# friendlymatthew/heif

Measured on AMD Instinct MI355X. Metric: Mpixels/s decoded (bit-exact) on 4032x3024 HEIC batch, higher is better.
Workload: dtype u8

## Files before the change

heif_amd/csrc/api.cpp:

```cpp
#include <hip/hip_runtime.h>

#include <algorithm>
#include <cmath>
#include <cstdlib>
#include <cstring>
#include <atomic>
#include <memory>
#include <mutex>
#include <string>
#include <thread>
#include <vector>

#include "../../include/heifgpu.h"
#include "common/desc.hpp"
#include "host/batch.hpp"
#include "host/heic_image.hpp"
#include "kernels/cabac.hpp"
#include "kernels/kernels.hpp"

using namespace hg;

struct heifgpu_image {
    ParsedImage img;
};
// ... 962 lines not shown
    b->cur = gi;
    b->loaded = true;
    BatchArgs &a = b->args;
    a = BatchArgs{};
    a.bits = b->bits.p;
    a.pics = G.pics.p;
    a.subs = b->subs.p;
    a.rbsp = nullptr;
    a.rsubs = nullptr;
    a.parse_order = b->porder.p;
    a.n_slots = int(order.size());
    a.parse_group = parse_group;
    a.seqs = G.seqs.p;
    a.sf = G.sf.p;
    a.outs = G.outs.p;
    a.recon = b->recon.p;
    a.n_pics = b->n_pics;
    a.max_width = hb.max_w;
    a.max_wctb = hb.max_wctb;
    a.max_rows = hb.max_rows;
    a.max_log2ctb = hb.max_log2ctb;
    a.lane_rows = hb.lane_rows;
    a.parse_mode = mode;
    a.solo_waves = solo_waves;
    a.xprog = nullptr;
    a.xctx = cross_rows ? b->xctx.p : nullptr;
    a.intra_stream = intra_stream_for(mode, int(hb.pics.size()), hb.has_assembly, ctx->stream) ? 1 : 0;
    a.xntu = nullptr;
    a.stream_patience_us = ctx->stream.patience_us;
    a.wpp_ring = mode == PARSE_SOLO ? (hb.max_wpp_rows > solo_waves ? 1 : 0) : hb.wpp_ring;
    a.lanes_lean = mode == PARSE_LANES
                       ? lanes_variant_for(hb.seqs.data(), hb.pics.data(), int(hb.pics.size()), a.wpp_ring)
                       : LANES_GENERAL;
    a.has_assembly = hb.has_assembly ? 1 : 0;
    a.total_rows = int(hb.rows);
    a.bytes_per_sample = hb.bps;
    a.chroma_format = hb.chroma;
    G.out_host.assign(n, OutImage{});
    if (fresh) *inout = fresh.release();
    return HEIFGPU_OK;
}

int heifgpu_batch_prepare(heifgpu_ctx *ctx, const heifgpu_image *const *imgs, size_t n, heifgpu_batch **out) {
    if (!out) return fail(HEIFGPU_E_INVALID, "invalid argument");
    *out = nullptr;
    const int rc = heifgpu_batch_prepare_ex(ctx, imgs, n, nullptr, out);
    if (rc) return rc;
    HIP_TRY(hipStreamSynchronize(ctx->upload));
    return HEIFGPU_OK;
}

int heifgpu_batch_decode(heifgpu_ctx *ctx, heifgpu_batch *b, const heifgpu_planes *out, void *stream) {
    if (!ctx || !b || !out) return fail(HEIFGPU_E_INVALID, "invalid argument");
    if (b->device != ctx->device) return fail(HEIFGPU_E_INVALID, "batch belongs to another device");
    if (!b->loaded) return fail(HEIFGPU_E_INVALID, "batch not loaded (its last prepare failed)");
    hipStream_t s = static_cast<hipStream_t>(stream);
    HIP_TRY(hipSetDevice(ctx->device));
    DescGen &G = b->gen[b->cur];
    bool changed = false;
    for (size_t i = 0; i < b->n_images; ++i) {
        OutImage o{};
        for (int c = 0; c < 3; ++c) {
            o.plane[c] = reinterpret_cast<uint64_t>(out[i].plane[c]);
            o.pitch[c] = out[i].pitch[c];
        }
        if (!out[i].plane[0] || (b->infos[i].chroma_format_idc && (!out[i].plane[1] || !out[i].plane[2])))
// ... 357 lines not shown
```

heif_amd/csrc/emu/emu_check.cpp:

```cpp
#include <cstdio>
#include <cstdlib>
#include <cstring>
#include <vector>

#include "../../../oracle/oracle.h"
#include "../host/batch.hpp"
#include "../kernels/cabac.hpp"
#include "../kernels/kernels.hpp"

namespace hg {
thread_local EmuCtx g_emu;
}
using namespace hg;

int main(int argc, char **argv) {
    if (argc < 2) return 2;
    setvbuf(stdout, nullptr, _IONBF, 0);
    int stages = argc > 2 ? atoi(argv[2]) : 5;
    const bool host_only = stages <= 0;
    const uint32_t tstride = !host_only && argc > 4 ? uint32_t(atoi(argv[3])) : 1u,
                   toff = !host_only && argc > 4 ? uint32_t(atoi(argv[4])) : 0u;
    auto read_file = [](const char *path, std::vector<uint8_t> &out) {
        FILE *f = fopen(path, "rb");
        if (!f) return false;
// ... 1 lines not shown
        long n = ftell(f);
        fseek(f, 0, SEEK_SET);
        out.assign(static_cast<size_t>(n), 0);
        const bool ok = fread(out.data(), 1, size_t(n), f) == size_t(n);
        fclose(f);
        return ok;
    };
    std::vector<uint8_t> data;
    if (!read_file(argv[1], data)) return 2;
    std::vector<std::vector<uint8_t>> more_data;
    for (int k = 3; host_only && k < argc; ++k) {
        more_data.emplace_back();
        if (!read_file(argv[k], more_data.back())) return 2;
    }
    ParsedImage im;
    std::vector<ParsedImage> more(more_data.size());
    HostBatch hb;
    try {
        im = parse_heic(data.data(), data.size());
        std::vector<const ParsedImage *> ims{&im};
        for (size_t k = 0; k < more.size(); ++k) {
            more[k] = parse_heic(more_data[k].data(), more_data[k].size());
            ims.push_back(&more[k]);
        }
        hb = build_batch(ims.data(), ims.size(), tstride, toff);
    } catch (const std::exception &e) {
        printf("host rejected: %s\n", e.what());
        return 3;
    }
    std::vector<TuRec> tus(hb.tu_n);
    std::vector<Coef> coefs(hb.coef_n);
    std::vector<uint32_t> rc(2 * hb.rows), status(hb.pics.size());
    std::vector<uint8_t> recon(hb.recon_bytes), maps(hb.map_bytes);
    std::vector<int16_t> resid(hb.resid_elems);
    std::vector<SaoParams> sao(hb.sao_n);
    const int W = int(im.out_width), H = int(im.out_height), bps = hb.bps;
    const int SX = chroma_sx(hb.chroma), SY = chroma_sy(hb.chroma);
    const int CW = (W + (1 << SX) - 1) >> SX, CH = (H + (1 << SY) - 1) >> SY;
    constexpr uint8_t kSentinel = 0xa5;
    std::vector<uint8_t> oy(size_t(W) * H * bps, kSentinel), ocb(size_t(CW) * CH * bps, kSentinel),
        ocr(size_t(CW) * CH * bps, kSentinel);
    OutImage out{};
    out.plane[0] = uint64_t(oy.data());
    out.plane[1] = uint64_t(ocb.data());
    out.plane[2] = uint64_t(ocr.data());
    out.pitch[0] = W * bps;
    out.pitch[1] = out.pitch[2] = CW * bps;
    out.width = W;
    out.height = H;
    BatchArgs a{};
    a.bits = hb.bits.data();
    a.pics = hb.pics.data();
    a.subs = hb.subs.data();
    std::vector<uint8_t> rbsp(hb.bits.size(), 0);
    std::vector<uint32_t> rsubs(hb.subs.size(), 0);
    a.rbsp = rbsp.data();
    a.rsubs = rsubs.data();
    std::vector<uint32_t> order;
    const int mode = parse_mode_for(PARSE_AUTO, int(hb.pics.size()), hb.pics.data());
    const int solo_waves = solo_waves_for(hb.lane_rows);
    int parse_group = 1;
    if (mode == PARSE_SPREAD) spread_parse_order(hb.pics.data(), int(hb.pics.size()), order);
    else
        parse_group = lanes_parse_order(hb.pics.data(), int(hb.pics.size()), hb.lane_rows, mode == PARSE_SOLO ? 1 : 0,
                                        order);
    std::vector<uint32_t> xprog(hb.rows + 1), xntu(hb.rows + hb.pics.size() + 1, 0);
// ... 1 lines not shown
    a.parse_order = order.data();
    a.n_slots = int(order.size());
    a.parse_group = parse_group;
    a.seqs = hb.seqs.data();
    a.sf = hb.sf.data();
    a.outs = &out;
    a.tus = tus.data();
    a.coefs = coefs.data();
    a.row_counts = rc.data();
    a.recon = recon.data();
    a.resid = resid.data();
    a.maps = maps.data();
    a.sao = sao.data();
    a.status = status.data();
    a.n_pics = int(hb.pics.size());
    a.max_width = hb.max_w;
    a.max_wctb = hb.max_wctb;
    a.max_rows = hb.max_rows;
    a.max_log2ctb = hb.max_log2ctb;
    a.lane_rows = hb.lane_rows;
    a.parse_mode = mode;
    a.solo_waves = solo_waves;
    a.xprog = xprog.data();
    a.xctx = xctx.data();
    a.xjob = xprog.data() + hb.rows;
    const StreamKnobs knobs = stream_knobs_from_env();
    a.intra_stream = intra_stream_for(mode, int(hb.pics.size()), hb.has_assembly, knobs) ? 1 : 0;
    a.xntu = a.intra_stream ? xntu.data() : nullptr;
    a.stream_patience_us = knobs.patience_us;
    a.wpp_ring = mode == PARSE_SOLO ? (hb.max_wpp_rows > solo_waves ? 1 : 0) : hb.wpp_ring;
    a.lanes_lean = mode == PARSE_LANES
                       ? lanes_variant_for(hb.seqs.data(), hb.pics.data(), int(hb.pics.size()), a.wpp_ring)
                       : LANES_GENERAL;
    a.has_assembly = hb.has_assembly ? 1 : 0;
    a.total_rows = int(hb.rows);
    a.bytes_per_sample = bps;
    a.chroma_format = hb.chroma;
    if (stages <= 0) {
        printf("host ok: %zu pictures\n", hb.pics.size());
        printf("parse mode: %s\n", mode == PARSE_SOLO ? "solo" : mode == PARSE_SPREAD ? "spread" : "lanes");
        if (mode == PARSE_LANES) printf("lanes variant: %s\n", a.lanes_lean ? "lean" : "general");
        return 0;
    }
    std::fill(rc.begin(), rc.end(), 0xa5a5a5a5u);
    std::fill(status.begin(), status.end(), 0x5au);
    std::fill(xprog.begin(), xprog.end(), 0x7777u);
    std::fill(xntu.begin(), xntu.end(), 0x3333u);
    emu_rbsp(a);
    emu_parse(a);
    uint32_t st = 0;
    for (uint32_t s : status) st |= s;
    uint64_t ntu = 0, ncoef = 0;
    for (uint32_t r = 0; r < hb.rows; ++r) {
        ntu += rc[2 * r];
        ncoef += rc[2 * r + 1];
    }
    if (getenv("HG_EMU_DEBUG_MODES")) {
        int shown = 0;
        for (const PicDesc &pd : hb.pics)
            for (uint32_t r = 0; r < (uint32_t)((hb.seqs[pd.seq].height + (1 << hb.seqs[pd.seq].log2_ctb) - 1) >> hb.seqs[pd.seq].log2_ctb); ++r) {
                const uint32_t nt = rc[2 * (pd.row_off + r)];
                for (uint32_t t = 0; t < nt && shown < 10; ++t) {
                    const TuRec &tu = tus[pd.tu_off + (uint64_t)r * pd.tu_cap_row + t];
                    if (tu.mode > 34) {
                        printf("bad mode %d pic %u row %u t %u x %d y %d log2 %d flags 0x%x ctu %d\n", tu.mode, (unsigned)(&pd - hb.pics.data()), r, t, tu.x, tu.y, tu.log2, tu.flags, tu.ctu);
                        ++shown;
                    }
                }
            }
    }
    printf("parse mode: %s\n", mode == PARSE_SOLO     ? "solo"
                               : mode == PARSE_SPREAD ? "spread"
                                                      : "lanes");
    if (mode == PARSE_LANES) printf("lanes variant: %s\n", a.lanes_lean ? "lean" : "general");
    printf("parse: status 0x%x, %llu TBs, %llu coefficients\n", st, (unsigned long long)ntu, (unsigned long long)ncoef);
    if (stages >= 2 && !a.intra_stream) emu_transform(a);
    if (stages >= 3) {
        emu_intra(a);
        if (a.intra_stream) {
            BatchArgs a2 = a;
            a2.stream_redo = 1;
            emu_intra(a2);
        }
    }
    if (stages >= 4) emu_deblock(a);
    if (stages >= 5) {
        emu_sao_out(a);
    } else {
        int dbk = stages >= 4 ? 0 : 1;
        oracle_set_debug_flags(dbk | 2);
        for (const PicDesc &pd : hb.pics) {
            const SeqParams &sp = hb.seqs[pd.seq];
            for (int c = 0; c < 3; ++c) {
                if (c && !sp.chroma_format) break;
                const int sx = c ? SX : 0, sy = c ? SY : 0, PW = sp.width >> sx, PH = sp.height >> sy;
                size_t off = c == 0 ? 0 : size_t(sp.width) * sp.height + size_t(c - 1) * PW * PH;
                int vw = std::min(sp.out_w, W - pd.out_x) >> sx, vh = std::min(sp.out_h, H - pd.out_y) >> sy;
                for (int y = 0; y < vh; ++y)
                    for (int x = 0; x < vw; ++x) {
                        size_t src = (off + size_t(y + (sp.conf_t >> sy)) * PW + x + (sp.conf_l >> sx)) * bps;
                        uint8_t *dst = reinterpret_cast<uint8_t *>(out.plane[c]) +
                                       size_t((pd.out_y >> sy) + y) * out.pitch[c] + size_t((pd.out_x >> sx) + x) * bps;
                        memcpy(dst, recon.data() + pd.recon_off + src, size_t(bps));
                    }
            }
        }
    }
    if (stages < 3) return st ? 1 : 0;
    oracle_image ref;
    if (oracle_decode_heic(data.data(), data.size(), &ref, nullptr, 0, nullptr)) {
        printf("oracle failed: %s\n", oracle_last_error());
        return 1;
    }
    long bad_total = 0;
    const char *names[3] = {"Y", "Cb", "Cr"};
    for (int c = 0; c < 3; ++c) {
        const uint8_t *g = c == 0 ? oy.data() : (c == 1 ? ocb.data() : ocr.data());
        int pw = int(ref.pw[c]), ph = int(ref.ph[c]);
// ... 28 lines not shown
```

heif_amd/csrc/emu/emu_parse.cpp:

```cpp
#include "../kernels/parse_units.hpp"

#include <cstdio>
#include <string>
#include <vector>

namespace hg {

template <class EG>
void emu_parse_lanes(const BatchArgs &a) {
    const int ppw = a.parse_order && a.parse_group > 0 ? a.parse_group : lanes_pics_per_wave(a.lane_rows, a.n_pics);
    const int n_slots = a.parse_order ? a.n_slots : a.n_pics;
    const int waves = (n_slots + ppw - 1) / ppw;
    uint64_t tab[kTabRows], seq[15];
    uint8_t scan8[128];
    for (int i = 0; i < 64; ++i) scan8_tables(scan8, i);
    for (int i = 0; i < kTabRows; ++i) tab[i] = state_row_ctx(i);
    for (int i = 0; i < 15; ++i) seq[i] = sig_seq(i);
    std::vector<LaneLds> lds(64);
    std::vector<LanePic> pics(64);
    std::vector<Lane> lanes(64);
    std::vector<uint8_t> wctx(a.wpp_ring ? 64 * CTX_PAD : 0);
    uint32_t prog[64];
    static const bool stats = std::getenv("HEIFGPU_LANES_STATS") != nullptr;
    static const std::string order = [] {
// ... 49 lines not shown
                    HG_COV(any4 ? COV_SB_RUN_ANY4 : COV_SB_RUN_NO4);
                }
                for (int l = 0; l < 64; ++l) {
                    Lane &L = lanes[l];
                    E.lane = l;
                    LanePic &P = pics[l / a.lane_rows];
                    if (!mine[l]) continue;
                    progressed = true;
                    ++units;
                    const EG G{lds[l].ctx, tab, seq, a.rbsp, (P.bits_end + 64u) & ~3u, scan8, scan8 + 64};
                    run_unit(kind, L, lds[l], P, E, G);
                }
            }
            if (!progressed) {
                for (int l = 0; l < 64; ++l)
                    if (lanes[l].st != U_DONE) {
                        lanes[l].status |= ST_SUBSTREAM_END;
                        atomicOr(&a.status[pics[l / a.lane_rows].pic], lanes[l].status & ~ST_SEGSW);
                        lanes[l].st = U_DONE;
                    }
                break;
            }
        }
        if (stats) {
            printf("wave %d: %ld passes, %.1f units per pass, %ld kind runs, %.2f units per kind run\n", w, passes,
                   (double)units / passes, kruns, (double)units / kruns);
            printf("  runs");
            for (int k = U_CTU; k <= U_TBD; ++k) printf(" %ld", kr[k]);
            printf("\n  units");
            for (int k = U_CTU; k <= U_TBD; ++k) printf(" %ld", ku[k]);
            printf("\n  paths");
            for (int k = 0; k < COV_N; ++k) printf(" %ld", g_cov[k]), g_cov[k] = 0;
            printf("\n  sb_paths");
            for (int k = COV_N; k < COV_ALL; ++k) printf(" %ld", g_cov[k]), g_cov[k] = 0;
            printf("\n");
        }
    }
}

template <bool Spread>
void emu_parse_solo(const BatchArgs &a) {
    using EG = EngSoloT<Spread>;
    const int NW = Spread ? a.max_rows : a.solo_waves;
    const int n_slots = a.parse_order ? a.n_slots : a.n_pics;
    uint64_t seq[15];
    for (int i = 0; i < 15; ++i) seq[i] = sig_seq(i);
    std::vector<LaneLds> lds((size_t)NW);
    std::vector<Lane> lanes((size_t)NW);
    std::vector<uint8_t> wctx((size_t)NW * CTX_PAD);
    std::vector<uint32_t> wbuf((size_t)NW * 192);
    std::vector<SoloWin> wins((size_t)NW);
    LanePic P;
    uint32_t prog[64];
    for (int slot = 0; slot < n_slots; ++slot) {
        const bool in = !a.parse_order || a.parse_order[slot] != ~0u;
        if (!in) continue;
        const uint32_t ent = a.parse_order ? a.parse_order[slot] : (uint32_t)slot;
        if (Spread && (ent >> 20) != 0) continue;
        const int pic = a.pic0 + (int)(Spread ? (ent & 0xfffffu) : ent);
        for (int w = 0; w < NW; ++w) {
            prog[w] = 0;
            if (!lane_init<false>(lanes[(size_t)w], P, lds[(size_t)w], a, pic, w, 0, Spread ? (1 << 20) : NW))
                lanes[(size_t)w].st = U_DONE;
            wins[(size_t)w].w = &wbuf[(size_t)w * 192];
            wins[(size_t)w].f = &wbuf[(size_t)w * 192 + 128];
        }
        const uint32_t lim = (P.bits_end + 64u) & ~3u;
// ... 43 lines not shown
```

heif_amd/csrc/kernels/kernels.hpp:

```cpp
#pragma once
#include "../common/desc.hpp"
#include "wave.hpp"
#include <cstdlib>
#include <vector>

#if defined(HG_HOST_EMU)
#include <atomic>
#include <thread>
#endif

namespace hg {

struct BatchArgs {
    const uint8_t *bits;
    const PicDesc *pics;
    const uint32_t *subs;
    uint8_t *rbsp;
    uint32_t *rsubs;
    const uint32_t *parse_order;
    int n_slots;
    const SeqParams *seqs;
    const uint8_t *sf;
    const OutImage *outs;
    TuRec *tus;
    Coef *coefs;
    uint32_t *row_counts;
    uint8_t *recon;
    int16_t *resid;
    uint8_t *maps;
    SaoParams *sao;
    uint32_t *status;
    int n_pics;
    int pic0;
    int max_width;
    int max_wctb;
    int max_rows;
    int total_rows;
    int bytes_per_sample;
    int chroma_format;
    int parse_group;
    int max_log2ctb;
    int lane_rows;
    int wpp_ring;
    int parse_mode;
    int solo_waves;
    uint32_t *xprog;
    uint8_t *xctx;
    uint32_t *xntu;
    uint32_t *xjob;
    int intra_stream;
    int stream_redo;
    uint32_t stream_patience_us;
    int has_assembly;
    int intra_split;
    int lanes_lean;
};

struct ColorArgs {
    uint64_t plane[3];
    int32_t pitch[3];
    uint64_t rgb;
    int32_t rgb_pitch;
    int32_t w, h;
    int32_t out_w, out_h;
    int32_t rotation;
    int32_t chroma, shift;
    int32_t yoff, ys;
    int32_t cr_r, cb_g, cr_g, cb_b;
};
struct GatherArgs {
    uint64_t dst[3], src[3];
    int32_t dpitch[3], spitch[3];
    int32_t planes, bps;
    int32_t sx, sy;
    int32_t W, H;
    int32_t tw, th, cols, n_tiles, stride, offset;
};
inline void color_coefs(uint32_t matrix, bool full, ColorArgs &c) {
    double kr = 0.299, kb = 0.114;
    if (matrix == 1) kr = 0.2126, kb = 0.0722;
    else if (matrix == 9) kr = 0.2627, kb = 0.0593;
    const double kg = 1.0 - kr - kb;
    const double ys = full ? 1.0 : 255.0 / 219.0, cs = full ? 1.0 : 255.0 / 224.0;
    auto fx = [](double v) { return (int32_t)(v * 65536.0 + 0.5); };
    c.yoff = full ? 0 : 16;
    c.ys = fx(ys);
    c.cr_r = fx(2.0 * (1.0 - kr) * cs);
    c.cb_b = fx(2.0 * (1.0 - kb) * cs);
// ... 142 lines not shown
```

heif_amd/csrc/kernels/parse_state.hpp:

```cpp
#pragma once
#include "cabac.hpp"
#include "kernels.hpp"
#include "tables.hpp"

#include <algorithm>
#include <cstdint>
#include <vector>

#if defined(HG_HOST_EMU)
#include <cstdio>
#endif

#if !defined(HG_HOST_EMU)
extern "C" __device__ int hg_writelane(int src, int lane, int old) __asm("llvm.amdgcn.writelane.i32");
#endif
#if !defined(HG_NO_COLD_HINTS)
#define HG_UNLIKELY(x) __builtin_expect(!!(x), 0)
#define HG_LIKELY(x) __builtin_expect(!!(x), 1)
#else
#define HG_UNLIKELY(x) (x)
#define HG_LIKELY(x) (x)
#endif

namespace hg {
// ... 89 lines not shown

struct Lane {
    uint32_t range, value;
    int k;
    uint64_t cur;
    int cn;
    uint32_t a0, a1, a2, a3, b0, b1, b2, b3, f0, f1, f2, f3;
    int ai, bv, fp;
    uint32_t lb;
    int32_t budget;
    uint32_t status;
    int st;
    uint32_t fl;
    int row, c, ctbx, ctby;
    int qx, qy, ql, qd;
    int tx, ty, tl, td;
    uint32_t tcbf;
    int qp_prev_last, qp_pred, cu_qp_delta_val, qpy_cur, qg_x, qg_y;
    int cu_modes, cu_chroma;
    int tb_t, tb_n, tb_cidx, tb_x, tb_y, tb_log2, tb_mode;
    uint32_t tb_coef0;
    int rc_scan, rc_last_sub, rc_last_pos, rc_i, rc_prev_c1;
    uint64_t rc_csbf;
    uint32_t ntu, ncoef;
    uint32_t nesc;
    uint32_t tu_row, coef_row;
    uint32_t cx;
    uint32_t reinit;
#if defined(HG_PARSE_PROF_SB)
    uint64_t psb[6];
#endif
};
#if defined(HG_PARSE_PROF_SB) && !defined(HG_HOST_EMU)
#define HG_SB_T(L, i, t0)                                                            \
    do {                                                                             \
        const uint64_t t_ = __builtin_amdgcn_s_memtime();                            \
        if ((int)__lane_id() == __builtin_ctzll(__ballot(1))) (L).psb[i] += t_ - (t0); \
        (t0) = t_;                                                                   \
    } while (0)
#else
#define HG_SB_T(L, i, t0) ((void)0)
#endif

enum Cov : int {
    COV_TB_LUMA,
    COV_TB_CHROMA = COV_TB_LUMA + 4,
    COV_NXN = COV_TB_CHROMA + 4,
    COV_NXN_MPM,
    COV_NXN_REM = COV_NXN_MPM + 3,
    COV_DQP,
    COV_DQP_EG0,
    COV_LAST_SUFFIX,
    COV_CODED_AFTER_EMPTY,
    COV_CU_ENDS_IN_SB,
    COV_TSKIP,
    COV_LAST_CTX5,
    COV_N,
    COV_SB_SIG4 = COV_N,
    COV_SB_SIG,
    COV_SB_BEYOND8,
    COV_SB_RICE4,
    COV_SB_ESCAPE,
    COV_SB_EGK,
    COV_SB_HIDE,
    COV_SB_NO_HIDE,
    COV_SB_CTXSET_INC,
    COV_SB_INFER_DC,
    COV_SB_LAST_POS0,
    COV_SB_GT2,
    COV_SB_RUN_ANY4,
    COV_SB_RUN_NO4,
    COV_ALL
};
#if defined(HG_HOST_EMU)
long g_cov[COV_ALL];
#define HG_COV(i) (++g_cov[i])
#else
#define HG_COV(i) ((void)0)
#endif

HG_HD inline size_t lane_blocks_bytes(int n) { return (sizeof(LaneLds) * (size_t)n + 15) & ~(size_t)15; }

#if !defined(HG_HOST_EMU) && defined(HG_PARSE_PROF)
int prof_read(uint64_t *out, int n) {
    uint64_t tmp[16] = {};
    if (hipMemcpyFromSymbol(tmp, HIP_SYMBOL(hg::g_prof_lanes), sizeof(tmp)) != hipSuccess) return -1;
    const uint64_t zero[16] = {};
    if (hipMemcpyToSymbol(HIP_SYMBOL(hg::g_prof_lanes), zero, sizeof(zero)) != hipSuccess) return -1;
#if defined(HG_PARSE_PROF_SB)
    const int head = 16;
#else
    const int head = 8;
#endif
    for (int k = 0; k < n && k < head; ++k) out[k] = tmp[k];
    if (n <= head) return n < head ? n : head;
    const size_t m = std::min((size_t)(n - head), (size_t)hg::kCtuTimeCap * 3);
    if (hipMemcpyFromSymbol(out + head, HIP_SYMBOL(hg::g_ctu_t), m * sizeof(uint64_t)) != hipSuccess) return -1;
    std::vector<uint64_t> z((size_t)hg::kCtuTimeCap * 3, 0);
    if (hipMemcpyToSymbol(HIP_SYMBOL(hg::g_ctu_t), z.data(), z.size() * sizeof(uint64_t)) != hipSuccess) return -1;
    return (int)(head + m);
}
#endif

}
// ... 2 lines not shown
```

heif_amd/csrc/kernels/parse_units.hpp:

```cpp
#pragma once
#include "parse_engine.hpp"

namespace hg {
namespace {

HG_HD inline int mode422(int m) {
    constexpr uint32_t t[9] = {0x02020100u, 0x05030202u, 0x0b0a0807u, 0x12100f0du, 0x16151413u,
                               0x18181717u, 0x1b1a1919u, 0x1d1c1c1bu, 0x001f1e1du};
    return (int)((t[m >> 2] >> (8 * (m & 3))) & 0xffu);
}

HG_HD inline int chroma_qp_map(int qpi, int chroma) {
    if (chroma != 1) return qpi < 51 ? qpi : 51;
    if (qpi < 30) return qpi;
    if (qpi > 43) return qpi - 6;
    return qpi < 34 ? qpi - 1 : 33 + ((qpi - 34) >> 1);
}

HG_HD inline void update_qpy(Lane &L, const LanePic &P) {
    L.qpy_cur = ((L.qp_pred + L.cu_qp_delta_val + 52 + 2 * P.qpbdY) % (52 + P.qpbdY)) - P.qpbdY;
}

HG_HD inline void derive_qp_pred(Lane &L, const LaneLds &ld, const LanePic &P) {
    int prev;
// ... 433 lines not shown
        if (nxn) HG_COV(p ? COV_NXN_MPM + mpm : COV_NXN_REM);
        const int xPb = L.qx + (i & 1) * pb, yPb = L.qy + (i >> 1) * pb;
        const int m = derive_luma_mode(L, ld, xPb, yPb, p, mpm, rem);
        modes |= m << (8 * i);
        const int nb = pb >> 2, by = (yPb - L.ctby) >> 2, bx = (xPb - L.ctbx) >> 2;
        for (int k = 0; k < nb; ++k) {
            ld.ipmL[by + k] = (uint8_t)m;
            ld.ipmA[bx + k] = (uint8_t)m;
        }
    }
    L.cu_modes = modes;
    if (HG_PIC_CHROMA(P)) {
        const int nc = HG_PIC_CHROMA(P) == 3 ? np : 1;
        int cms = 0;
        for (int i = 0; i < nc; ++i) {
            const int icpm = dec(L, G, CTX_CHROMA_MODE) ? (int)byp_bits(L, G, 2) : 4;
            const int lm = (modes >> (8 * i)) & 0xff;
            int cm;
            if (icpm == 4) {
                cm = lm;
            } else {
                cm = icpm == 0 ? 0 : (icpm == 1 ? 26 : (icpm == 2 ? 10 : 1));
                if (cm == lm) cm = 34;
            }
            if (HG_PIC_CHROMA(P) == 2) cm = mode422(cm);
            cms |= cm << (8 * i);
        }
        L.cu_chroma = nc == 1 ? (int)((uint32_t)cms * 0x01010101u) : cms;
    }
    L.tx = L.qx, L.ty = L.qy, L.tl = L.ql, L.td = 0, L.tcbf = 0;
    L.st = U_TT;
}

template <class EG>
HG_HD inline void unit_tt(Lane &L, LaneLds &ld, LanePic &P, const EG &G) {
    const bool nxn = (L.fl & F_NXN) != 0;
    const int max_depth = P.maxDepthIntra + (nxn ? 1 : 0);
    for (;;) {
        bool split;
        if (L.tl <= P.maxTb && L.tl > P.minTb && L.td < max_depth && !(nxn && L.td == 0))
            split = dec(L, G, CTX_SPLIT_TF + 5 - L.tl) != 0;
        else
            split = L.tl > P.maxTb || (nxn && L.td == 0);
        uint32_t cbf = 0;
        if ((L.tl > 2 && HG_PIC_CHROMA(P)) || HG_PIC_CHROMA(P) == 3) {
            const uint32_t pc = L.td == 0 ? 3u : (L.tcbf >> (4 * (L.td - 1))) & 3u;
            const bool two = HG_PIC_CHROMA(P) == 2 && (!split || L.tl == 3);
            if (pc & 1) {
                cbf |= (uint32_t)dec(L, G, CTX_CBF_CHROMA + L.td);
                if (two) cbf |= (uint32_t)dec(L, G, CTX_CBF_CHROMA + L.td) << 2;
            }
            if (pc & 2) {
                cbf |= (uint32_t)dec(L, G, CTX_CBF_CHROMA + L.td) << 1;
                if (two) cbf |= (uint32_t)dec(L, G, CTX_CBF_CHROMA + L.td) << 3;
            }
        }
        L.tcbf = (L.tcbf & ~(15u << (4 * L.td))) | (cbf << (4 * L.td));
        if (!split) break;
        --L.tl;
        ++L.td;
    }
    const uint32_t cbf = (L.tcbf >> (4 * L.td)) & 15u;
    L.fl &= ~F_CBF_L;
    if (dec(L, G, CTX_CBF_LUMA + (L.td == 0 ? 1 : 0))) L.fl |= F_CBF_L;
    const bool chroma4 = (HG_PIC_CHROMA(P) == 1 || HG_PIC_CHROMA(P) == 2) && L.tl == 2;
    const uint32_t pc = L.td > 0 ? (L.tcbf >> (4 * (L.td - 1))) & 15u : 0u;
    const bool cbf_c = HG_PIC_CHROMA(P) == 0 ? false : (chroma4 ? pc != 0 : cbf != 0);
    if (((L.fl & F_CBF_L) || cbf_c) && (pic_flags<EG>(P) & SP_CU_QP_DELTA) && !(L.fl & F_DQP_CODED)) {
// ... 2 lines not shown
            v = dec(L, G, CTX_CU_QP_DELTA);
            if (v) {
                uint32_t t = ctx_ld(L, G, CTX_CU_QP_DELTA + 1);
                while (v < 5 && dec_t(L, G, t & 0x7fu, t)) ++v;
                ctx_st(L, G, CTX_CU_QP_DELTA + 1, t & 0x7fu);
            }
        } else {
            while (v < 5 && dec(L, G, CTX_CU_QP_DELTA + (v == 0 ? 0 : 1))) ++v;
        }
        HG_COV(COV_DQP);
        if (v == 5) {
            HG_COV(COV_DQP_EG0);
            int ones = 0;
            bool bad = false;
            while (byp(L, G)) {
                if (++ones > 31) {
                    bad = true;
                    break;
                }
            }
            if (bad) L.status |= ST_SYNTAX;
            else v += (int)(((1u << ones) - 1u) + byp_bits(L, G, ones));
        }
        if (v && byp(L, G)) v = -v;
        const int vlo = -(26 + P.qpbdY / 2), vhi = 25 + P.qpbdY / 2;
        if (HG_UNLIKELY(v < vlo || v > vhi)) {
            L.status |= ST_SYNTAX;
            v = v < vlo ? vlo : vhi;
        }
        L.fl |= F_DQP_CODED;
        L.cu_qp_delta_val = v;
        update_qpy(L, P);
    }
    {
        const int nb = 1 << (L.tl - 2), gx0 = L.tx >> 2, gy0 = L.ty >> 2;
        const int wx = gx0 + nb <= P.w4 ? nb : P.w4 - gx0, hy = gy0 + nb <= P.h4 ? nb : P.h4 - gy0;
        const uint64_t nf = (lane_fl<EG>(L) & F_BYPASS) ? MF_NOFILT : 0;
        const uint64_t rep = 0x0101010101010101ull;
        for (int y = 0; y < hy; ++y) {
            uint8_t *row = P.gflags + (size_t)(gy0 + y) * P.w4 + gx0;
            const uint64_t h = (y == 0 ? (uint64_t)MF_EDGE_H : 0u) | nf;
            store_bytes(row, wx, (rep * h) | (uint64_t)MF_EDGE_V);
        }
    }
    const int blk = L.td == 0 ? 0 : (((L.tx >> L.tl) & 1) | (((L.ty >> L.tl) & 1) << 1));
    L.tb_n = (HG_PIC_CHROMA(P) != 0 && (!chroma4 || blk == 3)) ? (HG_PIC_CHROMA(P) == 2 ? 5 : 3) : 1;
    L.tb_t = 0;
    L.st = U_TB;
}

template <class EG>
HG_HD inline void tu_emit(Lane &L, const LanePic &P) {
    const uint32_t fl = lane_fl<EG>(L);
    int qp;
    if (L.tb_cidx == 0) {
        qp = L.qpy_cur + P.qpbdY;
    } else {
        const int off = L.tb_cidx == 1 ? P.cbOff : P.crOff;
        int qpi = L.qpy_cur + off;
        qpi = qpi < -P.qpbdC ? -P.qpbdC : (qpi > 57 ? 57 : qpi);
        qp = chroma_qp_map(qpi, HG_PIC_CHROMA(P)) + P.qpbdC;
    }
    uint32_t f = (uint32_t)L.tb_cidx;
    if (fl & F_TB_CBF) f |= TU_CBF;
    if (fl & F_TS) f |= TU_TSKIP;
    if (fl & F_BYPASS) f |= TU_BYPASS;
    if (fl & F_PCM) f |= TU_PCM | TU_BYPASS;
    if (L.tb_cidx == 0 && L.tb_log2 == 2) f |= TU_DST;
    if (HG_LIKELY(L.ntu < P.tu_cap)) {
        const uint32_t w0 = (uint32_t)L.tb_x | ((uint32_t)L.tb_y << 16);
        const uint32_t w1 = (uint32_t)L.tb_log2 | (f << 8) | ((uint32_t)L.tb_mode << 16) | ((uint32_t)(uint8_t)qp << 24);
        const uint32_t w3 = (L.ncoef - L.tb_coef0) | ((uint32_t)L.c << 16);
        if (pic_flags<EG>(P) & PF_COHERENT) store_tu_agent(P.tu_base + L.tu_row + L.ntu, w0, w1, L.tb_coef0, w3);
        else store_tu(P.tu_base + L.tu_row + L.ntu, w0, w1, L.tb_coef0, w3);
        ++L.ntu;
    } else {
        L.status |= ST_CAPACITY;
    }
}

HG_HD inline void cu_done(Lane &L, LaneLds &ld, LanePic &P);

template <class EG>
HG_HD inline void tb_done(Lane &L, LaneLds &ld, LanePic &P) {
    tu_emit<EG>(L, P);
    if (++L.tb_t < L.tb_n) {
        L.st = U_TB;
        return;
    }
    while (L.td > 0) {
        const int s = 1 << L.tl;
        const int b = ((L.tx >> L.tl) & 1) | (((L.ty >> L.tl) & 1) << 1);
        if (b < 3) {
            const int px = L.tx & ~(2 * s - 1), py = L.ty & ~(2 * s - 1);
            L.tx = px + ((b + 1) & 1) * s;
            L.ty = py + ((b + 1) >> 1) * s;
            L.st = U_TT;
            return;
        }
        L.tx &= ~(2 * s - 1);
        L.ty &= ~(2 * s - 1);
        ++L.tl;
        --L.td;
    }
    cu_done(L, ld, P);
}

HG_HD inline void cu_done(Lane &L, LaneLds &ld, LanePic &P) {
    {
        const int n = 1 << L.ql, nd = n >> 3;
        const int dy = (L.qy - L.ctby) >> 3, dx = (L.qx - L.ctbx) >> 3;
        for (int k = 0; k < nd; ++k) {
            ld.qL[dy + k] = (int8_t)L.qpy_cur;
            ld.qA[dx + k] = (int8_t)L.qpy_cur;
        }
        const int nb = n >> 2, gx0 = L.qx >> 2, gy0 = L.qy >> 2;
        const int wx = gx0 + nb <= P.w4 ? nb : P.w4 - gx0, hy = gy0 + nb <= P.h4 ? nb : P.h4 - gy0;
        for (int y = 0; y < hy; ++y) {
            int8_t *row = P.gqpy + (size_t)(gy0 + y) * P.w4 + gx0;
            store_bytes(reinterpret_cast<uint8_t *>(row), wx, 0x0101010101010101ull * (uint8_t)L.qpy_cur);
        }
        L.qp_prev_last = L.qpy_cur;
    }
    while (L.qd > 0) {
        const int s = 1 << L.ql;
        const int px = L.qx & ~(2 * s - 1), py = L.qy & ~(2 * s - 1);
        for (int b = (((L.qx >> L.ql) & 1) | (((L.qy >> L.ql) & 1) << 1)) + 1; b < 4; ++b) {
            const int cx = px + (b & 1) * s, cy = py + (b >> 1) * s;
            if (cx < P.W && cy < P.H) {
                L.qx = cx;
                L.qy = cy;
                L.st = U_CQT;
                return;
            }
        }
        L.qx = px;
        L.qy = py;
        ++L.ql;
        --L.qd;
    }
    L.st = U_CTU_END;
}

template <class EG>
HG_HD inline void unit_tb(Lane &L, LaneLds &ld, LanePic &P, const EG &G) {
    const int t = L.tb_t;
    const bool chroma4 = (HG_PIC_CHROMA(P) == 1 || HG_PIC_CHROMA(P) == 2) && L.tl == 2;
    const bool c422 = HG_PIC_CHROMA(P) == 2;
    const int comp = t == 0 ? 0 : (c422 ? 1 + ((t - 1) >> 1) : t), half = (c422 && t > 0) ? (t - 1) & 1 : 0;
    bool cbf;
    L.tb_cidx = comp;
    if (t == 0) {
        L.tb_x = L.tx;
        L.tb_y = L.ty;
        L.tb_log2 = L.tl;
        int k = 0;
        if (L.fl & F_NXN) {
            const int half = 1 << (L.ql - 1);
            k = ((L.ty - L.qy) >= half ? 2 : 0) + ((L.tx - L.qx) >= half ? 1 : 0);
        }
        L.tb_mode = (L.cu_modes >> (8 * k)) & 0xff;
        cbf = (L.fl & F_CBF_L) != 0;
    } else if (!chroma4) {
        L.tb_log2 = HG_PIC_CHROMA(P) == 3 ? L.tl : L.tl - 1;
        L.tb_x = L.tx >> HG_PIC_SUBX(P);
        L.tb_y = (L.ty >> HG_PIC_SUBY(P)) + (half << L.tb_log2);
        int k = 0;
        if (HG_PIC_CHROMA(P) == 3 && (L.fl & F_NXN)) {
            const int hp = 1 << (L.ql - 1);
            k = ((L.ty - L.qy) >= hp ? 2 : 0) + ((L.tx - L.qx) >= hp ? 1 : 0);
        }
        L.tb_mode = (L.cu_chroma >> (8 * k)) & 0xff;
        cbf = ((L.tcbf >> (4 * L.td + (comp - 1) + 2 * half)) & 1u) != 0;
    } else {
        const int s = 1 << (L.tl + 1);
        L.tb_x = (L.tx & ~(s - 1)) >> 1;
        L.tb_y = ((L.ty & ~(s - 1)) >> HG_PIC_SUBY(P)) + 4 * half;
        L.tb_log2 = 2;
        L.tb_mode = L.cu_chroma & 0xff;
        cbf = ((L.tcbf >> (4 * (L.td - 1) + (comp - 1) + 2 * half)) & 1u) != 0;
    }
    L.fl = (L.fl & ~(F_TS | F_TB_CBF)) | (cbf ? F_TB_CBF : 0u);
    L.tb_coef0 = L.ncoef;
    if (!cbf) {
        if constexpr (EG::kSolo) tb_done<EG>(L, ld, P);
        else L.st = U_TBD;
        return;
    }
    const int l2 = L.tb_log2, n = 1 << l2, cidx = comp;
    HG_COV((cidx ? COV_TB_CHROMA : COV_TB_LUMA) + l2 - 2);
    if (t == 1 && !(L.fl & F_CBF_L)) HG_COV(COV_CODED_AFTER_EMPTY);
    if ((pic_flags<EG>(P) & SP_TRANSFORM_SKIP) && !(L.fl & F_BYPASS) && l2 == 2 && dec(L, G, CTX_TS_FLAG + (cidx ? 1 : 0)))
        L.fl |= F_TS;
    if (L.fl & F_TS) HG_COV(COV_TSKIP);
    const int cmax = (l2 << 1) - 1;
    const int off = cidx == 0 ? 3 * (l2 - 2) + ((l2 - 1) >> 2) : 15;
    const int shift = cidx == 0 ? (l2 + 1) >> 2 : l2 - 2;
    int px = 0, py = 0;
    while (px < cmax && dec(L, G, CTX_LAST_X + off + (px >> shift))) ++px;
    while (py < cmax && dec(L, G, CTX_LAST_Y + off + (py >> shift))) ++py;
    int lx = px, ly = py;
    if (px > 3 || py > 3) HG_COV(COV_LAST_SUFFIX);
    if (px > 8 || py > 8) HG_COV(COV_LAST_CTX5);
    if (px > 3) {
        const int k = (px >> 1) - 1;
        lx = (1 << k) * (2 + (px & 1)) + (int)byp_bits(L, G, k);
    }
    if (py > 3) {
        const int k = (py >> 1) - 1;
        ly = (1 << k) * (2 + (py & 1)) + (int)byp_bits(L, G, k);
    }
    int scan = 0;
    if (l2 == 2 || (l2 == 3 && (cidx == 0 || HG_PIC_CHROMA(P) == 3))) {
        if (L.tb_mode >= 6 && L.tb_mode <= 14) scan = 2;
        else if (L.tb_mode >= 22 && L.tb_mode <= 30) scan = 1;
    }
    if (scan == 2) {
        const int tt = lx;
        lx = ly;
        ly = tt;
    }
    if (HG_UNLIKELY(lx >= n || ly >= n)) {
        L.status |= ST_SYNTAX;
        lx &= n - 1;
        ly &= n - 1;
    }
    const int sbl = l2 - 2, sbw = 1 << sbl;
    L.rc_scan = scan;
    L.rc_last_sub = scan_inv(G, sbl, scan, (ly >> 2) * sbw + (lx >> 2));
    L.rc_last_pos = scan_inv(G, 2, scan, (ly & 3) * 4 + (lx & 3));
    L.rc_csbf = 0;
    L.rc_prev_c1 = 1;
    L.fl &= ~F_ANY_SB;
    L.rc_i = L.rc_last_sub;
    L.st = U_SB;
}

template <bool Scalar = false>
HG_HD inline uint64_t spread16_nib(uint32_t m) {
#if !defined(HG_HOST_EMU) && defined(__HIP_DEVICE_COMPILE__)
    if constexpr (Scalar) {
        uint64_t x2, x4;
        asm("s_bitreplicate_b64_b32 %0, %1" : "=s"(x2) : "s"(uni32(m & 0xffffu)));
        asm("s_bitreplicate_b64_b32 %0, %1" : "=s"(x4) : "s"((uint32_t)x2));
        return x4 & 0x1111111111111111ull;
    }
#endif
    uint64_t x = m & 0xffffu;
    x = (x | (x << 24)) & 0x000000ff000000ffull;
    x = (x | (x << 12)) & 0x000f000f000f000full;
    x = (x | (x << 6)) & 0x0303030303030303ull;
    x = (x | (x << 3)) & 0x1111111111111111ull;
    return x;
}

template <class EG>
constexpr bool kSbVec = !EG::kSolo;

HG_HD inline uint64_t spread16_nib_halves(uint32_t m) {
    auto half = [](uint32_t x) {
        x = (x | (x << 12)) & 0x000f000fu;
        x = (x | (x << 6)) & 0x03030303u;
        x = (x | (x << 3)) & 0x11111111u;
        return x;
    };
    return (uint64_t)half(m & 0xffu) | ((uint64_t)half((m >> 8) & 0xffu) << 32);
}

// ... 132 lines not shown
            }
            if (nstart >= 0) {
                HG_COV(l2 == 2 ? COV_SB_SIG4 : COV_SB_SIG);
                if (infer_dc && sig == 0) {
                    HG_COV(COV_SB_INFER_DC);
                    sig |= 1u;
                } else {
                    sig |= dec_slot((int)(seq & 15u));
                }
            } else {
                HG_COV(COV_SB_LAST_POS0);
            }
        }
        auto cw = [&](int i, uint32_t v) { ctx_st(L, G, cbase + i, v & 0xffu); };
        if constexpr (kCc7) {
            if (l2 == 2) {
                for (int k = 0; k < 9; ++k) cw(k, (uint32_t)(cc >> (7 * k)) & 0x7fu);
            } else {
                cw(0, (uint32_t)cc & 0x7fu);
                cw(off, (uint32_t)(cc >> 7) & 0x7fu);
                cw(off + 1, (uint32_t)(cc >> 14) & 0x7fu);
                cw(off + 2, (uint32_t)(cc >> 21) & 0x7fu);
            }
        } else if (l2 == 2) {
            for (int k = 0; k < 4; ++k) cw(k, c0 >> (8 * k));
            for (int k = 0; k < 4; ++k) cw(4 + k, c1 >> (8 * k));
            cw(8, c2);
        } else {
            cw(0, c0);
            cw(off, c0 >> 8);
            cw(off + 1, c0 >> 16);
            cw(off + 2, c0 >> 24);
        }
#if defined(HG_PARSE_PROF_SB) && !defined(HG_HOST_EMU)
        L.psb[4] += (uint64_t)(nstart + 1);
#endif
        HG_SB_T(L, 1, tsb);
    }
    if (sig) {
        int ctx_set = (i == 0 || cidx > 0) ? 0 : 2;
        if ((L.fl & F_ANY_SB) && L.rc_prev_c1 == 0) {
            HG_COV(COV_SB_CTXSET_INC);
            ++ctx_set;
        }
        L.fl |= F_ANY_SB;
        int c1 = 1;
        uint32_t g1 = 0, g2 = 0;
        const int gbase = CTX_GT1 + ctx_set * 4 + (cidx ? 16 : 0);
        uint32_t gc = ctx_ld(L, G, gbase) | (ctx_ld(L, G, gbase + 1) << 8) | (ctx_ld(L, G, gbase + 2) << 16) |
                      (ctx_ld(L, G, gbase + 3) << 24);
        const int first_sig = 31 - __builtin_clz(sig & (0u - sig));
        const int last_sig = msb32(sig);
        int num_g1 = 0, last_g1 = -1;
        uint32_t beyond8 = sig;
        if constexpr (EG::kSolo) {
            uint32_t &m = beyond8;
            for (int j = 0; j < 8 && m; ++j) {
                const int nn = msb32(m);
                m ^= 1u << nn;
                const uint32_t gs = (uint32_t)(c1 < 3 ? c1 : 3) * 8u;
                uint32_t cs = (gc >> gs) & 0xffu;
                const uint32_t f = (uint32_t)dec_s(L, G, cs);
                gc = (gc & ~(0xffu << gs)) | (cs << gs);
                g1 |= f << nn;
                c1 = (c1 > 0 && !f) ? c1 + 1 : 0;
            }
            last_g1 = g1 ? msb32(g1) : -1;
// ... 290 lines not shown
```

heif_amd/csrc/kernels/transform.hip:

```cpp
#include "xform.hpp"

namespace hg {

namespace {

#ifndef HG_XF_WAVES
#define HG_XF_WAVES 4
#endif
constexpr int kWaves = HG_XF_WAVES;

#define wave_sync() HG_WAVE_SYNC()

}

#if !defined(HG_XF_WPE)
#define HG_XF_WPE 7
#endif
__global__ void __launch_bounds__(kWaves * 64) __attribute__((amdgpu_waves_per_eu(HG_XF_WPE))) k_transform(BatchArgs a) {
    HG_BLOCK_SHARED __attribute__((aligned(16))) int16_t dtile[kWaves][32 * kXfDStride32];
    HG_BLOCK_SHARED __attribute__((aligned(16))) int16_t gtile[kWaves][32 * 32];
    HG_BLOCK_SHARED int32_t extent[kWaves][2];
    HG_BLOCK_SHARED XfTab s_tab;
#if defined(HG_HOST_EMU)
    xf_tables(&s_tab, 0, 1);
// ... 140 lines not shown
                     res_plane[cidx] + (size_t)tu.y * pitch[cidx] + tu.x, pitch[cidx], lane);
    };
    auto wanted = [&](const TuRec &tu) {
        const int cidx = tu.flags & TU_CIDX_MASK, n = 1 << tu.log2;
        return (tu.flags & TU_CBF) && tu.log2 != 2 && tu.log2 <= 5 && cidx <= 2 && tu.x + n <= pitch[cidx] &&
               tu.y + n <= (cidx ? ch : H);
    };
#if defined(HG_HOST_EMU)
    for (uint32_t t = wave; t < ntu; t += kWaves)
        if (wanted(tus[t])) pass_b(tus[t]);
#else
    for (uint32_t t0 = wave; t0 < ntu; t0 += 64u * kWaves) {
        const uint32_t t = t0 + (uint32_t)lane * kWaves;
        uint4 rec = make_uint4(0, 0, 0, 0);
        if (t < ntu) rec = *reinterpret_cast<const uint4 *>(tus + t);
        TuRec mine;
        __builtin_memcpy(&mine, &rec, sizeof(mine));
        uint64_t todo = __ballot(t < ntu && wanted(mine));
        while (todo) {
            const int j = __builtin_ctzll(todo);
            todo &= todo - 1;
            const uint4 r = make_uint4((uint32_t)__builtin_amdgcn_readlane((int)rec.x, j),
                                       (uint32_t)__builtin_amdgcn_readlane((int)rec.y, j),
                                       (uint32_t)__builtin_amdgcn_readlane((int)rec.z, j),
                                       (uint32_t)__builtin_amdgcn_readlane((int)rec.w, j));
            TuRec tu;
            __builtin_memcpy(&tu, &r, sizeof(tu));
            pass_b(tu);
        }
    }
#endif
}

#if defined(HG_HOST_EMU)
void emu_transform(const BatchArgs &a) { emu_launch(k_transform, a.max_rows, a.n_pics, kWaves, a); }
#else
hipError_t launch_transform(const BatchArgs &a, hipStream_t s) {
    hipLaunchKernelGGL(k_transform, dim3(a.max_rows, a.n_pics), dim3(kWaves * 64), 0, s, a);
    return hipGetLastError();
}
#endif

}
```

Before: 26810.

## Move deblock edge-flag painting out of lanes parser into separate kernel

In the lanes parse mode the per-TU deblocking edge/bypass flag map is no longer written inside the serial CABAC parse loop. A new kernel launched after the transform pass rebuilds those flags from the stored TU records instead. The aim is to shorten the latency-bound parse critical path by moving byte-map stores into a parallel pass. The cost is an extra kernel launch and a re-read of the TU records, and the change also adds per-TB profiling macros and coverage counters for the emulator.

```diff
diff --git a/heif_amd/csrc/api.cpp b/heif_amd/csrc/api.cpp
--- a/heif_amd/csrc/api.cpp
+++ b/heif_amd/csrc/api.cpp
@@ -1018,6 +1018,7 @@
     a.lanes_lean = mode == PARSE_LANES
                        ? lanes_variant_for(hb.seqs.data(), hb.pics.data(), int(hb.pics.size()), a.wpp_ring)
                        : LANES_GENERAL;
+    a.flags_from_recs = mode == PARSE_LANES ? 1 : 0;
     a.has_assembly = hb.has_assembly ? 1 : 0;
     a.total_rows = int(hb.rows);
     a.bytes_per_sample = hb.bps;
diff --git a/heif_amd/csrc/emu/emu_check.cpp b/heif_amd/csrc/emu/emu_check.cpp
--- a/heif_amd/csrc/emu/emu_check.cpp
+++ b/heif_amd/csrc/emu/emu_check.cpp
@@ -57,6 +57,7 @@
     std::vector<Coef> coefs(hb.coef_n);
     std::vector<uint32_t> rc(2 * hb.rows), status(hb.pics.size());
     std::vector<uint8_t> recon(hb.recon_bytes), maps(hb.map_bytes);
+    if (getenv("HEIFGPU_EMU_DUMP_MAPS")) std::fill(maps.begin(), maps.end(), uint8_t(0xa5));
     std::vector<int16_t> resid(hb.resid_elems);
     std::vector<SaoParams> sao(hb.sao_n);
     const int W = int(im.out_width), H = int(im.out_height), bps = hb.bps;
@@ -124,6 +125,7 @@
     a.lanes_lean = mode == PARSE_LANES
                        ? lanes_variant_for(hb.seqs.data(), hb.pics.data(), int(hb.pics.size()), a.wpp_ring)
                        : LANES_GENERAL;
+    a.flags_from_recs = mode == PARSE_LANES ? 1 : 0;
     a.has_assembly = hb.has_assembly ? 1 : 0;
     a.total_rows = int(hb.rows);
     a.bytes_per_sample = bps;
@@ -176,6 +178,16 @@
         }
     }
     if (stages >= 4) emu_deblock(a);
+    if (const char *path = getenv("HEIFGPU_EMU_DUMP_MAPS")) {
+        FILE *f = fopen(path, "wb");
+        if (!f) return 2;
+        for (const PicDesc &pd : hb.pics) {
+            const SeqParams &sp = hb.seqs[pd.seq];
+            const size_t n = size_t((sp.width + 3) >> 2) * size_t((sp.height + 3) >> 2);
+            fwrite(maps.data() + pd.map_off, 1, 2 * n, f);
+        }
+        fclose(f);
+    }
     if (stages >= 5) {
         emu_sao_out(a);
     } else {
diff --git a/heif_amd/csrc/emu/emu_parse.cpp b/heif_amd/csrc/emu/emu_parse.cpp
--- a/heif_amd/csrc/emu/emu_parse.cpp
+++ b/heif_amd/csrc/emu/emu_parse.cpp
@@ -105,7 +105,9 @@
             printf("\n  paths");
             for (int k = 0; k < COV_N; ++k) printf(" %ld", g_cov[k]), g_cov[k] = 0;
             printf("\n  sb_paths");
-            for (int k = COV_N; k < COV_ALL; ++k) printf(" %ld", g_cov[k]), g_cov[k] = 0;
+            for (int k = COV_N; k < COV_SB_END; ++k) printf(" %ld", g_cov[k]), g_cov[k] = 0;
+            printf("\n  tb_paths");
+            for (int k = COV_SB_END; k < COV_ALL; ++k) printf(" %ld", g_cov[k]), g_cov[k] = 0;
             printf("\n");
         }
     }
diff --git a/heif_amd/csrc/kernels/kernels.hpp b/heif_amd/csrc/kernels/kernels.hpp
--- a/heif_amd/csrc/kernels/kernels.hpp
+++ b/heif_amd/csrc/kernels/kernels.hpp
@@ -54,6 +54,7 @@
     int has_assembly;
     int intra_split;
     int lanes_lean;
+    int flags_from_recs;
 };
 
 struct ColorArgs {
diff --git a/heif_amd/csrc/kernels/parse_state.hpp b/heif_amd/csrc/kernels/parse_state.hpp
--- a/heif_amd/csrc/kernels/parse_state.hpp
+++ b/heif_amd/csrc/kernels/parse_state.hpp
@@ -145,14 +145,26 @@
 #endif
 };
 #if defined(HG_PARSE_PROF_SB) && !defined(HG_HOST_EMU)
-#define HG_SB_T(L, i, t0)                                                            \
+#define HG_PHASE_T(L, i, t0)                                                         \
     do {                                                                             \
         const uint64_t t_ = __builtin_amdgcn_s_memtime();                            \
         if ((int)__lane_id() == __builtin_ctzll(__ballot(1))) (L).psb[i] += t_ - (t0); \
         (t0) = t_;                                                                   \
     } while (0)
+#endif
+#if defined(HG_PARSE_PROF_SB) && !defined(HG_HOST_EMU) && !defined(HG_PARSE_PROF_TB)
+#define HG_SB_T(L, i, t0) HG_PHASE_T(L, i, t0)
+#elif defined(HG_PARSE_PROF_TB) && !defined(HG_HOST_EMU)
+#define HG_SB_T(L, i, t0) ((void)(t0))
 #else
 #define HG_SB_T(L, i, t0) ((void)0)
+#endif
+#if defined(HG_PARSE_PROF_TB) && !defined(HG_HOST_EMU)
+#define HG_TB_T0(t0) uint64_t t0 = __builtin_amdgcn_s_memtime()
+#define HG_TB_T(L, i, t0) HG_PHASE_T(L, i, t0)
+#else
+#define HG_TB_T0(t0) ((void)0)
+#define HG_TB_T(L, i, t0) ((void)0)
 #endif
 
 enum Cov : int {
@@ -183,6 +195,14 @@
     COV_SB_GT2,
     COV_SB_RUN_ANY4,
     COV_SB_RUN_NO4,
+    COV_SB_END,
+    COV_LAST_00 = COV_SB_END,
+    COV_LAST_0M,
+    COV_LAST_M0,
+    COV_LAST_MM,
+    COV_LAST_SUFFIX_X_ONLY,
+    COV_LAST_SUFFIX_Y_ONLY,
+    COV_LAST_SWAP,
     COV_ALL
 };
 #if defined(HG_HOST_EMU)
diff --git a/heif_amd/csrc/kernels/parse_units.hpp b/heif_amd/csrc/kernels/parse_units.hpp
--- a/heif_amd/csrc/kernels/parse_units.hpp
+++ b/heif_amd/csrc/kernels/parse_units.hpp
@@ -489,8 +489,17 @@
     L.st = U_TT;
 }
 
+#if defined(HG_FLAGS_IN_PARSE)
+template <class EG>
+constexpr bool kFlagsInParse = true;
+#else
+template <class EG>
+constexpr bool kFlagsInParse = EG::kSolo;
+#endif
+
 template <class EG>
 HG_HD inline void unit_tt(Lane &L, LaneLds &ld, LanePic &P, const EG &G) {
+    HG_TB_T0(ttt);
     const bool nxn = (L.fl & F_NXN) != 0;
     const int max_depth = P.maxDepthIntra + (nxn ? 1 : 0);
     for (;;) {
@@ -559,7 +568,8 @@
         L.cu_qp_delta_val = v;
         update_qpy(L, P);
     }
-    {
+    HG_TB_T(L, 3, ttt);
+    if constexpr (kFlagsInParse<EG>) {
         const int nb = 1 << (L.tl - 2), gx0 = L.tx >> 2, gy0 = L.ty >> 2;
         const int wx = gx0 + nb <= P.w4 ? nb : P.w4 - gx0, hy = gy0 + nb <= P.h4 ? nb : P.h4 - gy0;
         const uint64_t nf = (lane_fl<EG>(L) & F_BYPASS) ? MF_NOFILT : 0;
@@ -570,6 +580,7 @@
             store_bytes(row, wx, (rep * h) | (uint64_t)MF_EDGE_V);
         }
     }
+    HG_TB_T(L, 4, ttt);
     const int blk = L.td == 0 ? 0 : (((L.tx >> L.tl) & 1) | (((L.ty >> L.tl) & 1) << 1));
     L.tb_n = (HG_PIC_CHROMA(P) != 0 && (!chroma4 || blk == 3)) ? (HG_PIC_CHROMA(P) == 2 ? 5 : 3) : 1;
     L.tb_t = 0;
@@ -634,6 +645,7 @@
 }
 
 HG_HD inline void cu_done(Lane &L, LaneLds &ld, LanePic &P) {
+    HG_TB_T0(tcu);
     {
         const int n = 1 << L.ql, nd = n >> 3;
         const int dy = (L.qy - L.ctby) >> 3, dx = (L.qx - L.ctbx) >> 3;
@@ -649,6 +661,7 @@
         }
         L.qp_prev_last = L.qpy_cur;
     }
+    HG_TB_T(L, 5, tcu);
     while (L.qd > 0) {
         const int s = 1 << L.ql;
         const int px = L.qx & ~(2 * s - 1), py = L.qy & ~(2 * s - 1);
@@ -671,6 +684,7 @@
 
 template <class EG>
 HG_HD inline void unit_tb(Lane &L, LaneLds &ld, LanePic &P, const EG &G) {
+    HG_TB_T0(ttb);
     const int t = L.tb_t;
     const bool chroma4 = (HG_PIC_CHROMA(P) == 1 || HG_PIC_CHROMA(P) == 2) && L.tl == 2;
     const bool c422 = HG_PIC_CHROMA(P) == 2;
@@ -724,11 +738,15 @@
     const int off = cidx == 0 ? 3 * (l2 - 2) + ((l2 - 1) >> 2) : 15;
     const int shift = cidx == 0 ? (l2 + 1) >> 2 : l2 - 2;
     int px = 0, py = 0;
+    HG_TB_T(L, 0, ttb);
     while (px < cmax && dec(L, G, CTX_LAST_X + off + (px >> shift))) ++px;
     while (py < cmax && dec(L, G, CTX_LAST_Y + off + (py >> shift))) ++py;
+    HG_TB_T(L, 1, ttb);
     int lx = px, ly = py;
     if (px > 3 || py > 3) HG_COV(COV_LAST_SUFFIX);
     if (px > 8 || py > 8) HG_COV(COV_LAST_CTX5);
+    if ((px == 0 || px == cmax) && (py == 0 || py == cmax)) HG_COV(COV_LAST_00 + (px ? 2 : 0) + (py ? 1 : 0));
+    if ((px > 3) != (py > 3)) HG_COV(px > 3 ? COV_LAST_SUFFIX_X_ONLY : COV_LAST_SUFFIX_Y_ONLY);
     if (px > 3) {
         const int k = (px >> 1) - 1;
         lx = (1 << k) * (2 + (px & 1)) + (int)byp_bits(L, G, k);
@@ -743,6 +761,7 @@
         else if (L.tb_mode >= 22 && L.tb_mode <= 30) scan = 1;
     }
     if (scan == 2) {
+        HG_COV(COV_LAST_SWAP);
         const int tt = lx;
         lx = ly;
         ly = tt;
@@ -761,6 +780,7 @@
     L.fl &= ~F_ANY_SB;
     L.rc_i = L.rc_last_sub;
     L.st = U_SB;
+    HG_TB_T(L, 2, ttb);
 }
 
 template <bool Scalar = false>
@@ -959,7 +979,7 @@
             cw(off + 1, c0 >> 16);
             cw(off + 2, c0 >> 24);
         }
-#if defined(HG_PARSE_PROF_SB) && !defined(HG_HOST_EMU)
+#if defined(HG_PARSE_PROF_SB) && !defined(HG_PARSE_PROF_TB) && !defined(HG_HOST_EMU)
         L.psb[4] += (uint64_t)(nstart + 1);
 #endif
         HG_SB_T(L, 1, tsb);
diff --git a/heif_amd/csrc/kernels/transform.hip b/heif_amd/csrc/kernels/transform.hip
--- a/heif_amd/csrc/kernels/transform.hip
+++ b/heif_amd/csrc/kernels/transform.hip
@@ -196,11 +196,53 @@
 #endif
 }
 
-#if defined(HG_HOST_EMU)
-void emu_transform(const BatchArgs &a) { emu_launch(k_transform, a.max_rows, a.n_pics, kWaves, a); }
+__global__ void __launch_bounds__(kWaves * 64) k_paint_flags(BatchArgs a) {
+    const int pic = a.pic0 + blockIdx.y, row = blockIdx.x;
+    const PicDesc pd = a.pics[pic];
+    if (pd.flags & PD_ASSEMBLY) return;
+    const SeqParams sp = a.seqs[pd.seq];
+    const int hctb = (sp.height + (1 << sp.log2_ctb) - 1) >> sp.log2_ctb;
+    if (row >= hctb) return;
+    const int w4 = (sp.width + 3) >> 2, h4 = (sp.height + 3) >> 2;
+    uint8_t *flg = a.maps + pd.map_off + (size_t)w4 * h4;
+    const uint32_t ntu = min(a.row_counts[2 * (pd.row_off + row)], pd.tu_cap_row);
+    const TuRec *tus = a.tus + pd.tu_off + (uint64_t)row * pd.tu_cap_row;
+    const int wave = (int)(threadIdx.x >> 6), lane = threadIdx.x & 63;
+    for (uint32_t t0 = 64u * wave; t0 < ntu; t0 += 64u * kWaves) {
+        for (int vl = lane; vl < 64; vl += kWave) {
+            const uint32_t t = t0 + (uint32_t)vl;
+            if (t >= ntu) continue;
+            const TuRec tu = tus[t];
+            if ((tu.flags & (TU_CIDX_MASK | TU_PCM)) || tu.log2 < 2 || tu.log2 > 5) continue;
+            const int nb = 1 << (tu.log2 - 2), gx0 = tu.x >> 2, gy0 = tu.y >> 2;
+            if (gx0 >= w4 || gy0 >= h4) continue;
+            const int wx = gx0 + nb <= w4 ? nb : w4 - gx0, hy = gy0 + nb <= h4 ? nb : h4 - gy0;
+            const uint8_t nf = (tu.flags & TU_BYPASS) ? MF_NOFILT : 0;
+            for (int y = 0; y < hy; ++y) {
+                uint8_t *r = flg + (size_t)(gy0 + y) * w4 + gx0;
+                const uint8_t h = (uint8_t)((y == 0 ? MF_EDGE_H : 0) | nf);
+                const uint64_t v = (0x0101010101010101ull * h) | (uint64_t)MF_EDGE_V;
+                if (wx == 8) {
+                    __builtin_memcpy(r, &v, 8);
+                } else if (wx == 4) {
+                    __builtin_memcpy(r, &v, 4);
+                } else {
+                    for (int x = 0; x < wx; ++x) r[x] = (uint8_t)(v >> (8 * x));
+                }
+            }
+        }
+    }
+}
+
+#if defined(HG_HOST_EMU)
+void emu_transform(const BatchArgs &a) {
+    emu_launch(k_transform, a.max_rows, a.n_pics, kWaves, a);
+    if (a.flags_from_recs) emu_launch(k_paint_flags, a.max_rows, a.n_pics, kWaves, a);
+}
 #else
 hipError_t launch_transform(const BatchArgs &a, hipStream_t s) {
     hipLaunchKernelGGL(k_transform, dim3(a.max_rows, a.n_pics), dim3(kWaves * 64), 0, s, a);
+    if (a.flags_from_recs) hipLaunchKernelGGL(k_paint_flags, dim3(a.max_rows, a.n_pics), dim3(kWaves * 64), 0, s, a);
     return hipGetLastError();
 }
 #endif
```

After: 27360, median of 6. 2.0% higher.
